# jthies/i-emic

Hardware: AMD Instinct MI355X
Metric: Newton-step wall time + SpMV achieved HBM GB/s, 2deg global ocean (lower is better)
Workload: dtype f64

## Files before the change

i-emic_amd/csrc/active_set.hip:

```cpp
#include <algorithm>
#include <vector>

#include "gs_internal.h"

namespace iemic {

namespace {

__global__ void k_cell_active(const uint8_t* __restrict__ known, Lay L, uint8_t* __restrict__ act)
{
    OWNED_CELL;
    bool a = false;
#pragma unroll
    for (int r = 0; r < NUN; r++) a |= !known[NUN * cell + r];
    act[lc] = a ? 1 : 0;
}

}

__global__ void k_dyn_pack(const double* __restrict__ val, const int* __restrict__ act, int64_t nact,
                           int64_t nloc, double* __restrict__ dvb, int64_t n)
{
    const int64_t t = (int64_t)blockIdx.x * blockDim.x + threadIdx.x;
    if (t >= n) return;
    const int64_t blk = t >> 12, s = (t >> 6) & 63, l = t & 63, h = blk * 64 + l;
    dvb[t] = h < nact ? val[s * nloc + act[h]] : 0.0;
}

__global__ void k_spmv_pack(const double* __restrict__ val, const int* __restrict__ act,
                                const int* __restrict__ apos, const int4* __restrict__ atl, int64_t nact,
                                int64_t nloc, double* __restrict__ spc)
{
    const int64_t t = (int64_t)blockIdx.x * blockDim.x + threadIdx.x;
    if (t >= (int64_t)NSLOT * nact) return;
    const int64_t s = t / nact, a = t - s * nact;
    const int4 td = atl[2 * apos[a]];
    spc[(int64_t)NSLOT * td.z + s * td.w + (a - td.z)] = val[s * nloc + act[a]];
}

__global__ void k_known_diff(const double* __restrict__ val, Lay L, int64_t rowintcon,
                             const uint8_t* __restrict__ known, double* __restrict__ nd)
{
    OWNED_CELL;
    int diff = 0;
    for (int r = 0; r < NUN; r++) {
        bool id = val[(int64_t)ROW_BEGIN[r] * ncell + lc] == 1.0;
        for (int s = ROW_BEGIN[r] + 1; id && s < ROW_BEGIN[r + 1]; s++)
            id = val[(int64_t)s * ncell + lc] == 0.0;
        const uint8_t k = (id && NUN * cell + r != rowintcon) ? 1 : 0;
        diff += k != known[NUN * cell + r];
    }
    if (diff) atomicAdd(nd, (double)diff);
}

static int act_tiles(iemic_ctx* c, const std::vector<uint8_t>& h, const std::vector<int>& cm)
{
    ActiveSet& as = c->gs.act;
    int rc;
    const int nx = c->sub.nx, tpr = (nx + 63) / 64;
    const int64_t nrow = c->sub.nloc / nx;
    std::vector<int> tl, ap((size_t)as.nact, 0);
    for (int64_t row = 0; row < nrow; row++)
        for (int ti = 0; ti < tpr; ti++) {
            const int i0 = ti * 64, nc = std::min(64, nx - i0);
            int lo = -1, hi = -1;
            uint64_t mask = 0;
            for (int cc = 0; cc < nc; cc++)
                if (h[row * nx + i0 + cc]) {
                    if (lo < 0) lo = cc;
                    hi = cc;
                    mask |= (uint64_t)1 << cc;
                }
            if (lo < 0) continue;
            const int a0 = cm[row * nx + i0 + lo], na = cm[row * nx + i0 + hi] - a0 + 1;
            for (int a = a0; a < a0 + na; a++) ap[a] = (int)(tl.size() / 8);
            tl.insert(tl.end(), {(int)(row * tpr + ti), lo | (hi << 8), a0, na, (int)(uint32_t)mask,
                                 (int)(uint32_t)(mask >> 32), 0, 0});
        }
    as.natile = (int)(tl.size() / 8);
    if (as.atl.reserve(tl.size() + 8)) return IEMIC_ENOMEM;
    if (!tl.empty() && (rc = h2d(c, as.atl.p, tl.data(), sizeof(int) * tl.size()))) return rc;
    if (as.apos.reserve(ap.size() + 1)) return IEMIC_ENOMEM;
    if (!ap.empty() && (rc = h2d(c, as.apos.p, ap.data(), sizeof(int) * ap.size()))) return rc;
    return 0;
}

int act_build(iemic_ctx* c, bool* changed)
{
    BlockGS& gs = c->gs;
    ActiveSet& as = gs.act;
    int rc;
    *changed = false;
    if (as.actf.reserve(c->sub.nloc)) return IEMIC_ENOMEM;
    hipLaunchKernelGGL(k_cell_active, dim3(blocks_for(c->sub.nloc)), dim3(256), 0, c->stream, gs.known.p,
                       lay_of(c->sub), as.actf.p);
    std::vector<uint8_t> h((size_t)c->sub.nloc);
    if ((rc = d2h(c, h.data(), as.actf.p, h.size()))) return rc;
    if (h == as.act_h) return 0;
    std::vector<int> list;
    list.reserve(h.size());
    for (int64_t q = 0; q < c->sub.nloc; q++)
        if (h[q]) list.push_back((int)q);
    as.nact = (int64_t)list.size();
    if (as.act.reserve(list.size() + 1)) return IEMIC_ENOMEM;
    if (!list.empty() && (rc = h2d(c, as.act.p, list.data(), sizeof(int) * list.size()))) return rc;
    std::vector<int> cm((size_t)c->sub.nloc, -1);
    for (size_t q = 0; q < list.size(); q++) cm[list[q]] = (int)q;
    if (as.cmap.reserve(cm.size())) return IEMIC_ENOMEM;
    if ((rc = h2d(c, as.cmap.p, cm.data(), sizeof(int) * cm.size()))) return rc;
    as.ric = -1;
    if (c->rowintcon >= 0) {
        const int64_t cell = c->rowintcon / NUN - c->sub.own0;
        if (cell >= 0 && cell < c->sub.nloc && cm[cell] >= 0) as.ric = (int64_t)NUN * cm[cell] + c->rowintcon % NUN;
    }
    if ((rc = act_tiles(c, h, cm))) return rc;
    as.act_h.swap(h);
    as.gen++;
    *changed = true;
    return 0;
}

static int dyn_halo_coefs(iemic_ctx* c)
{
    ActiveSet& as = c->gs.act;
    const int64_t row = (int64_t)c->l * c->sub.nx, nloc = c->sub.nloc;
    constexpr int NDS = 64;
    if (as.dvh.n < (size_t)(NDS * 2 * row)) {
        if (as.dvh.alloc((size_t)(NDS * 2 * row))) return IEMIC_ENOMEM;
        HIP_OK(hipMemsetAsync(as.dvh.p, 0, sizeof(double) * as.dvh.n, c->stream));
    }
    double* v = c->d_val.p;
    const int so = c->sub.nb[2], no = c->sub.nb[3];
    std::vector<Msg> y;
    push_pair(y, so, no, Seg{v, 0, NDS, row, nloc}, Seg{as.dvh.p, row, NDS, row, 2 * row},
              Seg{v, nloc - row, NDS, row, nloc}, Seg{as.dvh.p, 0, NDS, row, 2 * row});
    return run_msgs(c, y);
}

static int act_pack_dvb(iemic_ctx* c)
{
    ActiveSet& as = c->gs.act;
    if (as.nact <= 0 || !as.act.p) return 0;
    const int64_t nb = (as.nact + 63) / 64;
    if (as.dvb.reserve((size_t)(nb * 64 * 64))) return IEMIC_ENOMEM;
    hipLaunchKernelGGL(k_dyn_pack, dim3(blocks_for(nb * 64 * 64)), dim3(256), 0, c->stream, c->d_val.p,
                       (const int*)as.act.p, as.nact, c->sub.nloc, as.dvb.p, nb * 64 * 64);
    HIP_OK(hipGetLastError());
    return 0;
}

static int gs_pack_spc(iemic_ctx* c)
{
    ActiveSet& as = c->gs.act;
    if (as.nact <= 0 || !as.act.p) return 0;
    if (as.spc.reserve((size_t)(NSLOT * as.nact))) return IEMIC_ENOMEM;
    hipLaunchKernelGGL(k_spmv_pack, dim3(blocks_for(NSLOT * as.nact)), dim3(256), 0, c->stream, c->d_val.p,
                       (const int*)as.act.p, (const int*)as.apos.p, (const int4*)as.atl.p, as.nact, c->sub.nloc,
                       as.spc.p);
    HIP_OK(hipGetLastError());
    return 0;
}

int act_pack_streams(iemic_ctx* c)
{
    ActiveSet& as = c->gs.act;
    int rc;
    if (c->sub.nranks > 1 && c->sub.npx == 1 && (rc = dyn_halo_coefs(c))) return rc;
    if ((rc = act_pack_dvb(c))) return rc;
    if ((rc = gs_pack_spc(c))) return rc;
    as.vp = c->d_val.p;
    as.coef_stale = 0;
    as.cmp_ok = 1;
    return 0;
}

int gs_refresh(iemic_ctx* c)
{
    BlockGS& gs = c->gs;
    ActiveSet& as = gs.act;
    if (!as.coef_stale || !gs.ready || gs.kind != 2) return 0;
    as.coef_stale = 0;
    if (as.chk.reserve(1)) return IEMIC_ENOMEM;
    HIP_OK(hipMemsetAsync(as.chk.p, 0, sizeof(double), c->stream));
    hipLaunchKernelGGL(k_known_diff, dim3((unsigned)((c->sub.nloc + 255) / 256)), dim3(256), 0, c->stream,
                       c->d_val.p, lay_of(c->sub), (int64_t)c->rowintcon, gs.known.p, as.chk.p);
    int rc = allreduce_sum(c, as.chk.p, 1);
    if (rc) return rc;
    double nd = 0.0;
    if ((rc = d2h(c, &nd, as.chk.p, sizeof(double)))) return rc;
    if (nd != 0.0) as.cmp_ok = 0;
    return gs_pack_spc(c);
}

}
```

i-emic_amd/csrc/common.h:

```cpp
#ifndef IEMIC_COMMON_H
#define IEMIC_COMMON_H

#include <hip/hip_runtime.h>

#include <algorithm>
#include <cstdint>
#include <cstdio>
#include <string>
#include <vector>

#include "../../include/iemic.h"
#include "stencil.h"
#include "host_setup.h"
#include "decomp.h"

namespace iemic {

void set_error(const std::string& s);

#define HIP_OK(expr)                                                                   \
    do {                                                                               \
        hipError_t e_ = (expr);                                                        \
        if (e_ != hipSuccess) {                                                        \
            ::iemic::set_error(std::string(#expr) + ": " + hipGetErrorString(e_));     \
// ... 19 lines not shown
    }
    void free()
    {
        if (p) (void)hipFree(p);
        p = nullptr;
        n = 0;
    }
    DevBuf() = default;
    DevBuf(const DevBuf&) = delete;
    DevBuf& operator=(const DevBuf&) = delete;
    DevBuf(DevBuf&& o) noexcept : p(o.p), n(o.n) { o.p = nullptr; o.n = 0; }
    DevBuf& operator=(DevBuf&& o) noexcept
    {
        if (this != &o) {
            free();
            p = o.p; n = o.n;
            o.p = nullptr; o.n = 0;
        }
        return *this;
    }
    ~DevBuf() { free(); }
};

struct CrGemm {
    double* C;
    const double *C0, *C0b, *A1, *B1, *A2, *B2;
    double s1, s2;
};
constexpr int CR_MT = 8;
struct CrOut {
    int yb, nt;
    int64_t yo;
    double s[CR_MT];
    const double* A[CR_MT];
    int vb[CR_MT];
    int64_t vo[CR_MT];
};
struct CrComp {
    double* C;
    int nt;
    const double* A[4];
    const double* B[4];
    double s[4];
};
constexpr int CR_NCLS = 8;
struct CrCls {
    int ncls;
    int w0[CR_NCLS + 1];
    int nA[CR_NCLS];
    int64_t p0[CR_NCLS];
};
struct CrWg {
    int yref, r0;
    int nv, hasid;
    int vref[CR_MT];
};
struct CrPack {
    const double* A;
    double s;
    int64_t dst;
    int r0;
};
struct CrStep {
    int nwg = 0, rc = 16;
    int nl = 1;
    CrCls cls{};
    DevBuf<CrWg> wg;
    DevBuf<double> P;
    DevBuf<CrPack> jobs;
    int njobs = 0;
};
struct SchurCR {
    int n = 0, m = 0, periodic = 0, nlev = 0;
    std::vector<CrStep> down, up;
    DevBuf<double> cmat;
    DevBuf<CrComp> cdesc;
    int ncomp = 0;
    std::vector<int> N, per, merge;
    std::vector<size_t> dlr_off;
    std::vector<size_t> ap_off;
    std::vector<size_t> v_off;
    std::vector<int> g_off, g_cnt;
    int lt = 0, tM = 0;
    std::vector<size_t> tb_off;
    DevBuf<double> dlr, ap, bv, xv;
    DevBuf<double> tinv, tb, tx;
    DevBuf<CrGemm> gd;
    DevBuf<int> info;
};
int cr_init(iemic_ctx* c, SchurCR& cr, int n, int m, int periodic, int tail_max = 0);
int cr_factor(iemic_ctx* c, SchurCR& cr, const double* S9, const int* col_of_ij);
int cr_factor_blocks(iemic_ctx* c, SchurCR& cr);
int cr_check(iemic_ctx* c, SchurCR& cr);
int cr_solve(iemic_ctx* c, const SchurCR& cr, const double* b, double* x, hipStream_t s, double* xT = nullptr);
int cr_inverse_dev(hipStream_t s, int m, const double* src, double* dst, int* info);
int cr_inverse(hipStream_t s, int m, int count, const double* src, int s0, int sstep, double* dst, int* info);

struct TsMg {
    static constexpr int MAX = 12;
    int sweeps = 1, nlev = 0;
    int n[MAX] = {}, m[MAX] = {};
    int par[MAX] = {};
    DevBuf<double> off[MAX], diag[MAX], fac[MAX], b[MAX], z[MAX];
    DevBuf<double> zu[MAX];
    DevBuf<double> cinv;
    int glob = 0, gN = 0, gGX = 0, gI0 = 0, gJ0 = 0;
    DevBuf<double> gX, gband, gvec, gtmp, glpan;
    DevBuf<int> gpiv, ginfo, gcols;
    DevBuf<double> cdense;
    static constexpr int CR_CELLS = 1024;
    int crd = 0;
    int ckind = 0;
    bool nofuse = false;
    DevBuf<double> ep;
    DevBuf<uint64_t> etl;
    int64_t egen = -1, epn = 0;
    bool nopack = false;
    int hr = 0;
    SchurCR cr;
    DevBuf<int> cinfo;
};
int ts_mg_setup(iemic_ctx* c, int sweeps);
int ts_mg_solve(iemic_ctx* c, const double* zd, double* z, bool out, bool side);
int ts_mg_out(iemic_ctx* c, double* z);
int ts_mg_entry(iemic_ctx* c, const double* zd);
struct TsMgProbe {
    int nlev, lanes, sweeps, hr, ckind;
    int n, m, par, colours, fused, halo;
    const double *off, *diag, *b, *z, *cinv;
};
int ts_mg_probe(iemic_ctx* c, int q, TsMgProbe* o);

constexpr int BAND_NBP = 16;
int band_lu_inverse(iemic_ctx* c, double* ab, int N, int bl, int bu, int* piv, int* info_d, double* lpan,
                    const int* cols, double* X, int* info);

struct ActiveSet {
    DevBuf<int> act;
    DevBuf<int> cmap;
    int64_t ric = -1;
    DevBuf<uint8_t> actf;
    int64_t nact = 0;
    std::vector<uint8_t> act_h;
    int64_t gen = 0;
    DevBuf<double> spc;
    DevBuf<int> atl;
    DevBuf<int> apos;
    int natile = 0;
    DevBuf<double> dvh;
    DevBuf<double> dvb;
    const double* vp = nullptr;
    DevBuf<double> vold;
    int coef_stale = 0;
    int cmp_ok = 0;
    DevBuf<double> chk;
};
int act_build(iemic_ctx* c, bool* changed);
int act_pack_streams(iemic_ctx* c);
int gs_refresh(iemic_ctx* c);

struct TsSweeps {
    DevBuf<double> tsinv;
    DevBuf<double> tsoff;
    DevBuf<double> tsc, tic, bc;
    DevBuf<double> zt, zs;
    DevBuf<double> bts;
};

struct BlockGS {
    int ready = 0;
    int kind = 0;
    int ts_sweeps = 3;
    DevBuf<double> dinv;
    TsMg mg;
    ActiveSet act;
    TsSweeps sw;
    DevBuf<double> flags_d;
    std::vector<double> flags_h;
    DevBuf<int> own_pos;
    DevBuf<int> ocol;
    DevBuf<double> gslot;
    DevBuf<double> rcol;
    DevBuf<uint8_t> known;
    DevBuf<int> col_of_ij;
    DevBuf<int> ij_of_col;
    DevBuf<uint8_t> pinned;
    DevBuf<double> uvinv;
    DevBuf<double> tsdiag;
    DevBuf<double> pw;
    DevBuf<uint64_t> kmask;
    DevBuf<double> S9;
    SchurCR cr;
    int dyn_iters = 1;
    DevBuf<double> dres, zc;
    DevBuf<double> dq, dzero, dmr;
    int dyn_mr = 0;
    double dyn_omega = 1.0;
    int ts_at = 0;
    int schur_passes = 0;
    int ts_mg = 1;
    DevBuf<uint8_t> knP;
    DevBuf<double> zP, rrP;
    DevBuf<double> colvT;
    DevBuf<double> colvZ;
    DevBuf<double> rr, colv, colv2, colv_own;
};

struct Krylov {
    int m = 0;
    DevBuf<double> V, Z;
    DevBuf<double> w, r;
    int mc = 0;
    int64_t nc = 0;
    DevBuf<double> Vc, rf, t, bp;
    int zclean = 0;
};

struct Theta {
    double theta = 1.0, dt = 0.0;
    int init = 0;
    DevBuf<double> xold, Fold;
    DevBuf<double> Ft, b;
};

struct Eigs {
    int active = 0;
    int m = 0, j = 0;
    int broke = 0;
    double sigma = 0.0;
    DevBuf<double> V;
    DevBuf<double> t, w;
    DevBuf<double> lo;
};

constexpr int RED_BLOCKS = 1024;
__host__ __device__ inline double nanmax(double v, double a) { return (a > v || a != a) ? a : v; }
__device__ inline double block_nanmax(double v, double* sm)
{
    for (int o = 32; o > 0; o >>= 1) v = nanmax(v, __shfl_down(v, o, 64));
    if ((threadIdx.x & 63) == 0) sm[threadIdx.x >> 6] = v;
    __syncthreads();
    if (threadIdx.x == 0) {
        v = sm[0];
        for (int w = 1; w < 4; w++) v = nanmax(v, sm[w]);
    }
    return v;
}
constexpr int MAX_KRYLOV = 1000;
constexpr int RED_ROWS = 2 * MAX_KRYLOV + 8;
constexpr int DCGS_SCAL = 2 * MAX_KRYLOV + 2;

}

struct iemic_ctx {
    iemic_grid cfg;
    int device = 0;
    hipStream_t stream = nullptr;
    hipStream_t side = nullptr;
    hipEvent_t ev_fork = nullptr, ev_join = nullptr;
    int serial_setup = 0;
    int n = 0, m = 0, l = 0;
    int64_t ncell = 0, nrows = 0;
    int64_t rowintcon = -1;
    double int_correction = 0.0;
    void* comm = nullptr;
    void* group = nullptr;
    iemic_transport tp{};
    iemic::DevBuf<double> d_stage;
    std::vector<double> h_stage;
    int64_t stat[4] = {0, 0, 0, 0};
    double comm_timeout_s = 300.0;
    int comm_checked = 0;
    iemic::host::Setup su;
    const iemic::Sub& sub = su;
    iemic::DevBuf<int> d_landm;
    iemic::DevBuf<double> d_tab;
    iemic::DevBuf<double> d_ftab;
    iemic::DevBuf<double> d_frc;
    iemic::DevBuf<double> d_qcor;
    iemic::DevBuf<double> d_intc;
    iemic::DevBuf<double> d_atm;
    iemic::DevBuf<double> d_ins;
    int ins_on[4] = {0, 0, 0, 0};
    iemic::DevBuf<double> d_x, d_F, d_B, d_val;
    iemic::DevBuf<double> d_tmp1, d_tmp2, d_red;
    iemic::DevBuf<double> d_part, d_hbuf;
    double* h_red = nullptr;
    int jac_valid = 0;
    int refs = 1;
    iemic::BlockGS gs;
    iemic::Krylov kr;
    iemic::Theta th;
    iemic::Eigs eg;
    iemic::Geo geo() const;
    iemic_ctx() = default;
    iemic_ctx(const iemic_ctx&) = delete;
    iemic_ctx& operator=(const iemic_ctx&) = delete;
    ~iemic_ctx();
};

namespace iemic {
int dev_wait(iemic_ctx* c, hipEvent_t e, const char* what);
#define DEV_SYNC(c)                                                     \
    do {                                                                \
        const int rs_ = ::iemic::dev_wait((c), nullptr, __func__);      \
        if (rs_) return rs_;                                            \
    } while (0)
#define DEV_WAIT_EVENT(c, e)                                            \
    do {                                                                \
        const int rs_ = ::iemic::dev_wait((c), (e), __func__);          \
        if (rs_) return rs_;                                            \
    } while (0)
// ... 174 lines not shown
```

i-emic_amd/csrc/krylov.hip:

```cpp
#include <algorithm>
#include <cstdlib>
#include <chrono>
#include <cmath>

#include <hip/hip_ext.h>

#include "common.h"
#include "hessenberg.h"
#include "krylov_internal.h"
#include "vec_kernels.h"

namespace iemic {

__global__ void k_zero(double* __restrict__ p, int64_t n)
{
    for (int64_t q = (int64_t)blockIdx.x * blockDim.x + threadIdx.x; q < n; q += (int64_t)gridDim.x * blockDim.x)
        p[q] = 0.0;
}

__global__ void __launch_bounds__(256) k_mupdate_norm(const double* __restrict__ V, int64_t ldv,
                                                      int nvec, const double* __restrict__ h,
                                                      double* __restrict__ w, int64_t N,
                                                      double* __restrict__ partial)
{
// ... 337 lines not shown
        x[q] = acc;
    }
}

int mdot_host(iemic_ctx* c, const double* V, int64_t ldv, int nvec, const double* w,
              double* out, const double* ea, const double* eb)
{
    const int64_t N = c->sub.nlrows();
    const int nout = nvec + (ea ? 1 : 0);
    hipLaunchKernelGGL(k_mdot, dim3(RED_BLOCKS, nout), dim3(256), 0, c->stream, V, ldv, nvec, w, N,
                       c->d_part.p, ea, eb);
    hipLaunchKernelGGL(k_mdot_final, dim3(nout), dim3(256), 0, c->stream, c->d_part.p, RED_BLOCKS,
                       nout, c->d_hbuf.p);
    int rc = allreduce_sum(c, c->d_hbuf.p, nout);
    if (rc) return rc;
    HIP_OK(hipMemcpyAsync(c->h_red, c->d_hbuf.p, sizeof(double) * nout, hipMemcpyDeviceToHost,
                          c->stream));
    DEV_SYNC(c);
    for (int i = 0; i < nout; i++) out[i] = c->h_red[i];
    return 0;
}

int dot_owned(iemic_ctx* c, const double* a, const double* b, double* out)
{
    const int64_t o = owned(c).o;
    return mdot_host(c, a + o, 0, 1, b + o, out);
}

double dot(iemic_ctx* c, const double* a, const double* b, int64_t)
{
    const int64_t o = owned(c).o;
    double r = 0.0;
    if (mdot_host(c, a + o, 0, 1, b + o, &r)) return NAN;
    return r;
}

static int orth_pass(iemic_ctx* c, const double* V, int64_t ldv, int nvec, double* w, double* h,
                     double* ww0, double* ww1)
{
    const int64_t N = c->sub.nlrows();
    hipLaunchKernelGGL(k_mdot, dim3(RED_BLOCKS, nvec + 1), dim3(256), 0, c->stream, V, ldv, nvec,
                       w, N, c->d_part.p, (const double*)w);
    hipLaunchKernelGGL(k_mdot_final, dim3(nvec + 1), dim3(256), 0, c->stream, c->d_part.p,
                       RED_BLOCKS, nvec + 1, c->d_hbuf.p);
    int rc = allreduce_sum(c, c->d_hbuf.p, nvec + 1);
    if (rc) return rc;
    hipLaunchKernelGGL(k_mupdate_norm, dim3(RED_BLOCKS), dim3(256), 0, c->stream, V, ldv, nvec,
                       c->d_hbuf.p, w, N, c->d_part.p);
    hipLaunchKernelGGL(k_mdot_final, dim3(1), dim3(256), 0, c->stream, c->d_part.p, RED_BLOCKS, 1,
                       c->d_hbuf.p + nvec + 1);
    if ((rc = allreduce_sum(c, c->d_hbuf.p + nvec + 1, 1))) return rc;
    HIP_OK(hipMemcpyAsync(c->h_red, c->d_hbuf.p, sizeof(double) * (nvec + 2), hipMemcpyDeviceToHost,
                          c->stream));
    DEV_SYNC(c);
    for (int i = 0; i < nvec; i++) h[i] = c->h_red[i];
    *ww0 = c->h_red[nvec];
    *ww1 = c->h_red[nvec + 1];
    return 0;
}

int ensure_krylov(iemic_ctx* c, int m, int64_t nc)
{
    Krylov& k = c->kr;
    const int64_t N = c->sub.nerows();
    int rc = 0;
    if (k.m < m || !k.Z.p) {
        k.zclean = 0;
        k.V.free();
        rc |= k.Z.alloc((size_t)m * N);
        rc |= k.w.alloc(N);
        rc |= k.r.alloc(N);
        if (rc) {
            set_error("fgmres: out of device memory for the Krylov basis");
            return IEMIC_ENOMEM;
        }
        k.m = m;
    }
    if (!nc && !k.V.p) {
        if (k.V.alloc((size_t)(k.m + 1) * N)) {
            set_error("fgmres: out of device memory for the Krylov basis");
            return IEMIC_ENOMEM;
        }
    }
    if (nc && (k.mc < m || k.nc < nc || !k.Vc.p)) {
        rc |= k.Vc.alloc((size_t)(m + 1) * nc);
        if (!k.t.p) rc |= k.t.alloc(N) | k.bp.alloc(N);
        if (rc) {
            set_error("fgmres: out of device memory for the Krylov basis");
            return IEMIC_ENOMEM;
        }
        k.mc = m;
        k.nc = nc;
    }
    return 0;
}

__global__ void k_cgather(const double* __restrict__ full, const int* __restrict__ act, int64_t nc,
                          int64_t own0, double s, double* __restrict__ cmp)
{
    for (int64_t q = (int64_t)blockIdx.x * blockDim.x + threadIdx.x; q < nc;
         q += (int64_t)gridDim.x * blockDim.x) {
        const int64_t cl = q / NUN;
        cmp[q] = s * full[NUN * (own0 + act[cl]) + (q - NUN * cl)];
    }
}
__global__ void k_known_part(const double* __restrict__ v, const uint8_t* __restrict__ known, int64_t n0,
                             int64_t nl, double* __restrict__ t)
{
    for (int64_t q = (int64_t)blockIdx.x * blockDim.x + threadIdx.x; q < nl;
         q += (int64_t)gridDim.x * blockDim.x) {
        const int64_t r = n0 + q;
        t[r] = known[r] ? v[r] : 0.0;
    }
}

int upload_coeffs(iemic_ctx* c, const double* h, int n)
{
    if (n > RED_ROWS) {
        set_error("upload_coeffs: too many coefficients");
        return IEMIC_EINVAL;
    }
    double* st = c->h_red + RED_ROWS;
    for (int i = 0; i < n; i++) st[i] = h[i];
    HIP_OK(hipMemcpyAsync(c->d_hbuf.p + RED_ROWS, st, sizeof(double) * n,
                          hipMemcpyHostToDevice, c->stream));
    return 0;
}

int nonfinite()
{
    set_error("FGMRES: non-finite value in the Krylov basis (operator or preconditioner output)");
    return IEMIC_ERANGE;
}

double ms_since(std::chrono::steady_clock::time_point t0)
{
    return std::chrono::duration<double, std::milli>(std::chrono::steady_clock::now() - t0).count();
}

int prec_safeguard(iemic_ctx* c);

constexpr double STAG_RATIO = 0.25;
constexpr int STAG_MIN = 20;

int fgmres(iemic_ctx* c, const double* b, double* x, const iemic_krylov* opt, iemic_solve_info* info)
{
    const int m = std::max(1, std::min(opt->krylov_dim, MAX_KRYLOV));
    const Owned ow = owned(c);
    const int64_t NE = c->sub.nerows(), o = ow.o, NL = ow.n;
    const BlockGS& gs = c->gs;
    int rc = opt->prec > 0 ? gs_refresh(c) : 0;
    if (rc) return rc;
    const bool cmp = opt->orth == 0 && opt->prec == 2 && gs.ready && gs.kind == 2 && gs.act.nact > 0 && gs.act.cmap.p &&
                     gs.act.cmp_ok && gs.act.spc.p && gs.act.atl.p;
    const int64_t NC = cmp ? NUN * gs.act.nact : 0;
    rc = ensure_krylov(c, m, NC);
    if (rc) return rc;
    if (cmp && c->kr.zclean < m) {
        const int z0 = c->kr.zclean;
        if ((rc = dev_zero(c, c->kr.Z.p + (int64_t)z0 * NE, (int64_t)(m - z0) * NE))) return rc;
        c->kr.zclean = m;
    } else if (!cmp) {
        c->kr.zclean = 0;
    }
    iemic_solve_info inf{};
    auto T0 = std::chrono::steady_clock::now();
    double* V = cmp ? nullptr : c->kr.V.p;
    double* Vc = cmp ? c->kr.Vc.p : nullptr;
    double* Z = c->kr.Z.p;
    double* w = c->kr.w.p;
    double* r = c->kr.r.p;
    const unsigned G = ow.grid;
    const unsigned GC = grid_for(NC);
    Hessenberg hess(m);
    std::vector<double> h(m + 1), h2(m + 1), y(m);
    std::vector<double> zs(m + 1, 1.0);
    if (2 * m + 5 > RED_ROWS) {
        set_error("fgmres: Krylov dimension too large");
        return IEMIC_EINVAL;
    }
    int inf_reorth = 0;
    struct Events {
        hipEvent_t e[8] = {};
        ~Events() { for (auto& x : e) if (x) (void)hipEventDestroy(x); }
    } evs;
    hipEvent_t* ev = evs.e;
    hipEvent_t* evr = evs.e + 6;
    for (int q = 0; q < 6; q++) HIP_OK(hipEventCreate(&ev[q]));
    for (int q = 6; q < 8; q++) HIP_OK(hipEventCreateWithFlags(&evs.e[q], hipEventDisableTiming));

    if ((rc = dev_zero(c, x, NE))) return rc;
    double bnorm = sqrt0(dot(c, b, b, 0));
    if (!std::isfinite(bnorm)) return nonfinite();
    if (!(bnorm > 0)) {
        inf.converged = 1;
        if (info) *info = inf;
        return 0;
    }
    const double* b_orig = b;
    bool known_rhs = false;
    if (cmp) {
        double* t = c->kr.t.p;
        hipLaunchKernelGGL(k_known_part, dim3(G), dim3(256), 0, c->stream, b, gs.known.p, o, NL, t);
        if (dot(c, t, t, 0) > 0.0) {
            known_rhs = true;
            if ((rc = spmv(c, t, w, c->stream))) return rc;
            hipLaunchKernelGGL(k_axpby, dim3(G), dim3(256), 0, c->stream, 1.0, b + o, -1.0, w + o,
                               c->kr.bp.p + o, NL);
            b = c->kr.bp.p;
        }
    }
    HIP_OK(hipMemcpyAsync(r, b, sizeof(double) * NE, hipMemcpyDeviceToDevice, c->stream));
    double beta = known_rhs ? sqrt0(dot(c, b, b, 0)) : bnorm, res = beta / bnorm, res_c0 = res;
    int it = 0;
    struct Restore {
        iemic_ctx* c;
        int mr;
        ~Restore() { c->gs.dyn_mr = mr; }
    } restore{c, c->gs.dyn_mr};
    for (int cycle = 0; beta > 0.0 && cycle <= opt->max_restarts; cycle++) {
        const int it_c0 = it;
        if (cmp)
            hipLaunchKernelGGL(k_cgather, dim3(GC), dim3(256), 0, c->stream, r, gs.act.act.p, NC, c->sub.own0,
                               1.0 / beta, Vc);
        else
            hipLaunchKernelGGL(k_scale_copy, dim3(G), dim3(256), 0, c->stream, r + o, 1.0 / beta, V + o, NL);
        hess.reset(beta);
        int j = 0;
        if (opt->orth == 1) {
            for (; j < m; j++) {
                double* vj = V + (int64_t)j * NE;
                double* zj = Z + (int64_t)j * NE;
                double* vn = V + (int64_t)(j + 1) * NE;
                HIP_OK(hipEventRecord(ev[0], c->stream));
                if (opt->prec > 0) {
                    rc = prec_apply(c, vj, zj);
                    if (rc) return rc;
                } else {
                    HIP_OK(hipMemcpyAsync(zj, vj, sizeof(double) * NE, hipMemcpyDeviceToDevice, c->stream));
                }
                HIP_OK(hipEventRecord(ev[1], c->stream));
                rc = spmv(c, zj, vn, c->stream);
                if (rc) return rc;
                HIP_OK(hipEventRecord(ev[2], c->stream));

                double hn2 = 0.0;
                {
                    double ww0 = 0.0;
                    rc = orth_pass(c, V + o, NE, j + 1, vn + o, h.data(), &ww0, &hn2);
                    if (rc) return rc;
                    if (hn2 < 0.5 * ww0) {
                        double dummy = 0.0;
                        rc = orth_pass(c, V + o, NE, j + 1, vn + o, h2.data(), &dummy, &hn2);
                        if (rc) return rc;
                        for (int i = 0; i <= j; i++) h[i] += h2[i];
                        inf_reorth++;
                    }
                }
                if (!std::isfinite(hn2)) return nonfinite();
                double hn = sqrt0(hn2);
                if (hn > 0)
                    hipLaunchKernelGGL(k_scale_copy, dim3(G), dim3(256), 0, c->stream, vn + o, 1.0 / hn,
                                       vn + o, NL);
                {
                    float a1 = 0.f, a2 = 0.f;
                    (void)hipEventElapsedTime(&a1, ev[0], ev[1]);
                    (void)hipEventElapsedTime(&a2, ev[1], ev[2]);
                    inf.t_prec_ms += a1;
                    inf.t_spmv_ms += a2;
                    inf.n_spmv++;
                }
                res = hess.push_column(j, h.data(), hn) / bnorm;
                it++;
                if (res <= opt->tol || hn == 0.0) {
                    j++;
                    break;
                }
            }
        } else {
            std::vector<double> htent(m + 1), col(m + 1);
            int ncolf = 0;
            double* const Q = cmp ? Vc : V + o;
            const int64_t LQ = cmp ? NC : NE, NQ = cmp ? NC : NL;
            const int nbx1 = (int)std::min<int64_t>(RED_BLOCKS, (NQ / 2 + 256 * DOT1_E - 1) / (256 * DOT1_E));
            std::fill(zs.begin(), zs.end(), 1.0);
            auto enqueue = [&](int jj) -> int {
                double* u = Q + (int64_t)jj * LQ;
                double* wv = jj < m ? Q + (int64_t)(jj + 1) * LQ : nullptr;
                hipEvent_t* e = ev + 3 * (jj & 1);
                int rc2;
                if (jj < m) {
                    double* zj = Z + (int64_t)jj * NE;
                    HIP_OK(hipEventRecord(e[0], c->stream));
                    if (cmp) {
                        if ((rc2 = gs_apply_c(c, u, zj, jj > 0))) return rc2;
                    } else if (opt->prec > 0) {
                        if ((rc2 = prec_apply(c, u - o, zj))) return rc2;
                    } else {
                        HIP_OK(hipMemcpyAsync(zj, u - o, sizeof(double) * NE, hipMemcpyDeviceToDevice,
                                              c->stream));
                    }
                    if (cmp) {
                        if ((rc2 = halo_exchange(c, zj, 1))) return rc2;
                        if ((rc2 = spmv_kernel_c(c, zj, wv, e[1], e[2]))) return rc2;
                    } else {
                        HIP_OK(hipEventRecord(e[1], c->stream));
                        if ((rc2 = spmv(c, zj, wv - o, c->stream))) return rc2;
// ... 113 lines not shown
```

i-emic_amd/csrc/spmv.hip:

```cpp
#include <algorithm>
#include <cstdlib>

#include <hip/hip_ext.h>

#include "common.h"
#include "vec_kernels.h"

namespace iemic {

constexpr int SP7_T = 64;
__host__ __device__ constexpr int sp7_row(int s)
{
    return s < 24 ? 0 : s < 46 ? 1 : s < 53 ? 2 : s < 64 ? 3 : s < 84 ? 4 : 5;
}
__host__ __device__ constexpr int sp7_combo(int dj, int dk)
{
    return dk == 0 ? (dj + 1) : (dk == -1 ? (dj == 0 ? 3 : 5) : 4);
}
template <int S0, int S1>
__device__ __forceinline__ void sp7_load(const double* __restrict__ val, int64_t nloc, int64_t lc, bool act,
                                         double* v)
{
    if (act) {
#pragma unroll
        for (int s = S0; s < S1; s++) v[s - S0] = __builtin_nontemporal_load(val + (int64_t)s * nloc + lc);
    }
}
template <int S0, int S1>
__device__ __forceinline__ void sp7_compute(const double* v, const double* xs, int c, double* acc)
{
#pragma unroll
    for (int s = S0; s < S1; s++) {
        const Slot sl = SLOTS[s];
        const int q = sp7_combo(sl.dj, sl.dk);
        acc[sp7_row(s) - sp7_row(S0)] += v[s - S0] * xs[(q * (SP7_T + 2) + (c + 1 + sl.di)) * NUN + sl.var];
    }
}
__global__ void __launch_bounds__(256) k_spmv7(SubLay X, const double* __restrict__ val,
                                               const double* __restrict__ x,
                                               double* __restrict__ y, int nloc, int ntile, int tpr)
{
    __shared__ double xs[6 * (SP7_T + 2) * NUN];
    __shared__ double red[4][3][SP7_T];
    const int l = X.l, nx = X.nx;
    const int per = (ntile + 7) >> 3;
    const int tile = (int)(blockIdx.x & 7) * per + (int)(blockIdx.x >> 3);
    if (tile >= ntile) return;
    const int row = tile / tpr, i0 = (tile - row * tpr) * SP7_T;
    const int k = row % l, jl = row / l, j = X.jb0 + jl;
    const int nc = min(SP7_T, nx - i0);
    const int lc0 = row * nx + i0;
    const int t = threadIdx.x, c = t & 63;
    const int g = __builtin_amdgcn_readfirstlane(t >> 6);
    const bool act = c < nc;
    const int64_t lc = lc0 + c;
    double acc[3] = {0.0, 0.0, 0.0};
    double v[26];
    if (g == 0) sp7_load<0, 26>(val, nloc, lc, act, v);
    else if (g == 1) sp7_load<26, 52>(val, nloc, lc, act, v);
    else if (g == 2) sp7_load<52, 78>(val, nloc, lc, act, v);
    else sp7_load<78, 104>(val, nloc, lc, act, v);
    {
        const int jm = j > 0 ? j - 1 : j, jp = j < X.m - 1 ? j + 1 : j;
        const int km = k > 0 ? k - 1 : k, kp = k < l - 1 ? k + 1 : k;
        const int rj[6] = {jm, j, jp, j, j, jp}, rk[6] = {k, k, k, km, kp, km};
        constexpr int PR = (SP7_T + 2) * NUN;
        constexpr int SPT = (6 * PR + 255) / 256;
        const int lim = (nc + 2) * NUN;
        double xv[SPT];
        int xo[SPT];
#pragma unroll
        for (int u = 0; u < SPT; u++) {
            const int e = t + 256 * u;
            const int q = e / PR, w = e - q * PR;
            xo[u] = -1;
            if (e < 6 * PR && w < lim) {
                const int p = w / NUN, var = w - p * NUN;
                const int64_t r = (int64_t)(rj[q] - X.jb0 + HALO) * l + rk[q];
                const int64_t cell = (p == 0 || p == nc + 1)
                                         ? xnb_cell(r, i0 + p - 1, X.n, X.ib0, nx, X.hx, X.periodic, X.xb)
                                         : r * nx + i0 + p - 1;
                xo[u] = e;
                xv[u] = x[NUN * cell + var];
            }
        }
#pragma unroll
        for (int u = 0; u < SPT; u++)
            if (xo[u] >= 0) xs[xo[u]] = xv[u];
    }
    __syncthreads();
    if (g == 0) sp7_compute<0, 26>(v, xs, c, acc);
    else if (g == 1) sp7_compute<26, 52>(v, xs, c, acc);
    else if (g == 2) sp7_compute<52, 78>(v, xs, c, acc);
    else sp7_compute<78, 104>(v, xs, c, acc);
#pragma unroll
    for (int q = 0; q < 3; q++) red[g][q][c] = acc[q];
    __syncthreads();
    for (int o = t; o < nc * NUN; o += 256) {
        const int cc = o / NUN, R = o - cc * NUN;
        double v;
        switch (R) {
        case 0: v = red[0][0][cc]; break;
        case 1: v = red[0][1][cc] + red[1][0][cc]; break;
        case 2: v = red[1][1][cc] + red[2][0][cc]; break;
        case 3: v = red[2][1][cc]; break;
        case 4: v = red[2][2][cc] + red[3][0][cc]; break;
        default: v = red[3][1][cc]; break;
        }
        y[NUN * ((int64_t)HALO * l * nx + lc0) + o] = v;
    }
}

typedef __attribute__((address_space(3))) void lds_void;
typedef __attribute__((address_space(1))) void glb_void;
__global__ void __launch_bounds__(256) k_spmv7c(SubLay X, const double* __restrict__ spc,
                                                const double* __restrict__ x, double* __restrict__ y,
                                                const int4* __restrict__ atl, int natile, int tpr)
{
    __shared__ double xs[6 * (SP7_T + 2) * NUN];
    __shared__ double red[4][3][SP7_T];
    __shared__ int lof[SP7_T];
    const int l = X.l, nx = X.nx;
    const int per = (natile + 7) >> 3;
    const int pos = (int)(blockIdx.x & 7) * per + (int)(blockIdx.x >> 3);
    if (pos >= natile) return;
    const int4 td = atl[2 * pos], tm = atl[2 * pos + 1];
    const int tile = td.x, clo = td.y & 255, chi = td.y >> 8, a0 = td.z;
    const uint64_t amask = (uint64_t)(uint32_t)tm.x | ((uint64_t)(uint32_t)tm.y << 32);
    const int row = tile / tpr, i0 = (tile - row * tpr) * SP7_T;
    const int k = row % l, jl = row / l, j = X.jb0 + jl;
    const int nc = min(SP7_T, nx - i0);
    const int t = threadIdx.x, c = t & 63;
    const int g = __builtin_amdgcn_readfirstlane(t >> 6);
    const bool act = (amask >> c) & 1;
    const int cm = act ? a0 + __builtin_popcountll(amask & ((1ull << c) - 1)) : -1;
    if (g == 0 && act) lof[cm - a0] = c;
    double acc[3] = {0.0, 0.0, 0.0};
    double v[26];
    const double* vb = spc + (int64_t)NSLOT * a0;
    const int64_t vs = td.w, vo = cm - a0;
    if (g == 0) sp7_load<0, 26>(vb, vs, vo, act, v);
    else if (g == 1) sp7_load<26, 52>(vb, vs, vo, act, v);
    else if (g == 2) sp7_load<52, 78>(vb, vs, vo, act, v);
    else sp7_load<78, 104>(vb, vs, vo, act, v);
    {
        const int jm = j > 0 ? j - 1 : j, jp = j < X.m - 1 ? j + 1 : j;
        const int km = k > 0 ? k - 1 : k, kp = k < l - 1 ? k + 1 : k;
        const int rj[6] = {jm, j, jp, j, j, jp}, rk[6] = {k, k, k, km, kp, km};
        const int lane = t & 63, nb = nc * NUN * 8;
        const int blo = max(0, (clo - 1) * NUN * 8), bhi = min(nb, (chi + 2) * NUN * 8);
        for (int u = g; u < 18; u += 4) {
            const int q = u / 3, h = u - 3 * q;
            if (h * 1024 >= bhi || (h + 1) * 1024 <= blo) continue;
            const int byte = h * 1024 + lane * 16;
            const int64_t r = (int64_t)(rj[q] - X.jb0 + HALO) * l + rk[q];
            if (byte < nb)
                __builtin_amdgcn_global_load_lds((glb_void*)(x + NUN * (r * nx + i0) + byte / 8),
                                                 (lds_void*)(xs + (q * (SP7_T + 2) + 1) * NUN + h * 128), 16, 0, 0);
    }
        if (t < 72) {
            const int q = t / 12, side = (t / NUN) & 1, var = t - NUN * (t / NUN);
            const int p = side ? nc + 1 : 0;
            const int64_t r = (int64_t)(rj[q] - X.jb0 + HALO) * l + rk[q];
            const int64_t cell = xnb_cell(r, i0 + p - 1, X.n, X.ib0, nx, X.hx, X.periodic, X.xb);
            xs[(q * (SP7_T + 2) + p) * NUN + var] = x[NUN * cell + var];
    }
    }
    __syncthreads();
    if (act) {
        if (g == 0) sp7_compute<0, 26>(v, xs, c, acc);
        else if (g == 1) sp7_compute<26, 52>(v, xs, c, acc);
        else if (g == 2) sp7_compute<52, 78>(v, xs, c, acc);
        else sp7_compute<78, 104>(v, xs, c, acc);
    }
#pragma unroll
    for (int q = 0; q < 3; q++) red[g][q][c] = acc[q];
    __syncthreads();
    const int na = td.w;
    for (int o = t; o < na * NUN; o += 256) {
        const int ac = o / NUN, R = o - ac * NUN;
        const int cc = lof[ac];
        double vv;
        switch (R) {
        case 0: vv = red[0][0][cc]; break;
        case 1: vv = red[0][1][cc] + red[1][0][cc]; break;
        case 2: vv = red[1][1][cc] + red[2][0][cc]; break;
        case 3: vv = red[2][1][cc]; break;
        case 4: vv = red[2][2][cc] + red[3][0][cc]; break;
        default: vv = red[3][1][cc]; break;
        }
        y[(int64_t)NUN * a0 + o] = vv;
    }
}

template <int S0, int S1>
__device__ __forceinline__ void dyn_partial(const double* __restrict__ val, const double* __restrict__ z,
                                            int64_t vs, const int (*nc)[9], const bool* on,
                                            int64_t ps, double* acc)
{
    constexpr int NS = S1 - S0;
    double v[NS], zz[NS];
#pragma unroll
    for (int s = 0; s < NS; s++) v[s] = zz[s] = 0.0;
#pragma unroll
    for (int q = 0; q < 2; q++) {
        if (!on[q]) continue;
#pragma unroll
        for (int s = S0; s < S1; s++) {
            const Slot sl = SLOTS[s];
            if (sp7_row(s) - sp7_row(S0) != q) continue;
            const int cidx = nc[sl.di + 1][(sl.dk + 1) * 3 + (sl.dj + 1)];
            v[s - S0] = val[(int64_t)s * vs];
            zz[s - S0] = z[(int64_t)cidx + ps * sl.var];
        }
    }
#pragma unroll
    for (int s = S0; s < S1; s++) {
        const int q = sp7_row(s) - sp7_row(S0);
        if (on[q]) acc[q] += v[s - S0] * zz[s - S0];
    }
}
__global__ void __launch_bounds__(256) __attribute__((amdgpu_waves_per_eu(5, 8))) k_spmv_dyn(SubLay X, const double* __restrict__ val,
                                                  const double* __restrict__ z,
                                                  const double* __restrict__ r,
                                                  const uint8_t* __restrict__ knP,
                                                  double* __restrict__ d, int64_t nloc, int nblk, int64_t ps,
                                                  const double* __restrict__ hv, int nhb, int hs, int hn,
                                                  const int* __restrict__ alist, int64_t nown,
                                                  const double* __restrict__ vb)
{
    __shared__ double red[4][2][64];
    __shared__ int64_t us[64];
    __shared__ int oks[64];
    const int ntot = nblk + nhb;
    const int per = (ntot + 7) >> 3;
    const int tile = (int)(blockIdx.x & 7) * per + (int)(blockIdx.x >> 3);
    if (tile >= ntot) return;
    const int c = threadIdx.x & 63, g = threadIdx.x >> 6;
    const int64_t row = (int64_t)X.l * X.nx;
    const int64_t e0 = (int64_t)HALO * row;
    const bool halo = tile >= nblk;
    int64_t h, u;
    bool act;
    if (!halo) {
        h = (int64_t)tile * 64 + c;
        act = h < nown;
        u = !act ? 0 : (alist ? (int64_t)alist[h] : h);
    } else {
        h = (int64_t)(tile - nblk) * 64 + c;
        const bool south = h < row;
        act = h < 2 * row && (south ? hs : hn);
        u = south ? h - row : nloc + h - row;
    }
    if (g == 0) {
        us[c] = u;
        oks[c] = act ? 1 : 0;
    }
    double acc[2] = {0.0, 0.0};
    if (act) {
        const int64_t q = u + row;
        const int il = (int)(q % X.nx), k = (int)((q / X.nx) % X.l);
        const int j = X.jb0 - 1 + (int)(q / row);
        int nc[3][9];
        nb_cells(X, il, j, k, nc);
        const int64_t cell = e0 + u;
        const int v0 = g == 0 ? 0 : g - 1;
        const bool on[2] = {!knP[cell + ps * v0], g > 0 && !knP[cell + ps * (v0 + 1)]};
        const double* vp = halo ? hv + h : (vb ? vb + (int64_t)tile * 4096 + c : val + u);
        const int64_t vs = halo ? 2 * row : (vb ? 64 : nloc);
        if (g == 0) dyn_partial<0, 16>(vp, z, vs, nc, on, ps, acc);
        else if (g == 1) dyn_partial<16, 32>(vp, z, vs, nc, on, ps, acc);
        else if (g == 2) dyn_partial<32, 48>(vp, z, vs, nc, on, ps, acc);
        else dyn_partial<48, 64>(vp, z, vs, nc, on, ps, acc);
    }
    red[g][0][c] = acc[0];
    red[g][1][c] = acc[1];
    __syncthreads();
    const int R = threadIdx.x >> 6, cc = threadIdx.x & 63;
    if (!oks[cc]) return;
    const double sum = R == 0 ? red[0][0][cc] + red[1][0][cc]
                     : R == 1 ? red[1][1][cc] + red[2][0][cc]
                     : R == 2 ? red[2][1][cc] + red[3][0][cc]
                              : red[3][1][cc];
    const int64_t cell = e0 + us[cc], e = cell + ps * R;
    d[e] = knP[e] ? 0.0 : r[e] - sum;
}

int spmv_dyn_defect(iemic_ctx* c, const double* z, const double* r, const uint8_t* knP, double* d, bool halo)
{
    const BlockGS& gs = c->gs;
    const bool al = gs.act.act.p && gs.act.nact > 0;
    const int64_t nown = al ? gs.act.nact : c->sub.nloc;
    const int nblk = (int)((nown + 63) / 64);
    const int64_t row = (int64_t)c->l * c->sub.nx;
    const bool hv = halo && gs.act.dvh.p;
    const int nhb = hv ? (int)((2 * row + 63) / 64) : 0;
    const unsigned grid = 8u * (unsigned)((nblk + nhb + 7) / 8);
    hipLaunchKernelGGL(k_spmv_dyn, dim3(grid), dim3(256), 0, c->stream, sub_lay(c->sub), gs.act.vp, z, r, knP, d,
                       c->sub.nloc, nblk, (int64_t)c->sub.next, hv ? gs.act.dvh.p : nullptr, nhb,
                       hv && c->sub.nb[2] >= 0 ? 1 : 0, hv && c->sub.nb[3] >= 0 ? 1 : 0,
                       al ? gs.act.act.p : nullptr, nown, al && gs.act.dvb.p ? gs.act.dvb.p : nullptr);
    return 0;
}

static int spmv_intcond(iemic_ctx* c, const double* x, double* yr);
int spmv_kernel(iemic_ctx* c, const double* x, double* y)
{
    if (!c->jac_valid) {
        set_error("spmv: no Jacobian assembled");
        return IEMIC_ESTATE;
    }
    hipStream_t s = c->stream;
    if (c->sub.nloc >= INT32_MAX) {
        set_error("spmv: more than 2^31 cells per rank");
        return IEMIC_EINVAL;
    }
    const int tpr = (c->sub.nx + SP7_T - 1) / SP7_T;
    const int ntile = (int)(c->sub.nloc / c->sub.nx) * tpr;
    const unsigned grid = 8u * (unsigned)((ntile + 7) / 8);
    hipLaunchKernelGGL(k_spmv7, dim3(grid), dim3(256), 0, s, sub_lay(c->sub), c->d_val.p, x, y, (int)c->sub.nloc, ntile,
                       tpr);
    return spmv_intcond(c, x, c->rowintcon >= 0 ? y + c->rowintcon : nullptr);
}

static int spmv_intcond(iemic_ctx* c, const double* x, double* yr)
{
    hipStream_t s = c->stream;
    if (c->su.rowintcon_ref >= 0) {
        const Owned w = owned(c);
        hipLaunchKernelGGL(k_mdot, dim3(RED_BLOCKS, 1), dim3(256), 0, s, c->d_intc.p + w.o, (int64_t)0, 1,
                           x + w.o, w.n, c->d_red.p);
        hipLaunchKernelGGL(k_mdot_final, dim3(1), dim3(256), 0, s, c->d_red.p, RED_BLOCKS, 1,
                           c->d_red.p + RED_BLOCKS);
        int rc = allreduce_sum(c, c->d_red.p + RED_BLOCKS, 1);
        if (rc) return rc;
        if (c->rowintcon >= 0)
            hipLaunchKernelGGL(k_scale_copy, dim3(1), dim3(1), 0, s, c->d_red.p + RED_BLOCKS,
                               (double)c->cfg.int_sign, yr, (int64_t)1);
    }
    HIP_OK(hipGetLastError());
    return 0;
}

int spmv_kernel_c(iemic_ctx* c, const double* x, double* yc, hipEvent_t ev0, hipEvent_t ev1)
{
    const BlockGS& gs = c->gs;
    if (!c->jac_valid || !gs.act.cmap.p || !gs.act.spc.p || !gs.act.atl.p || gs.act.coef_stale) {
        set_error("spmv: no Jacobian, no active-cell map or stale packed coefficients");
        return IEMIC_ESTATE;
    }
    hipStream_t s = c->stream;
    const int tpr = (c->sub.nx + SP7_T - 1) / SP7_T;
    const unsigned grid = 8u * (unsigned)((gs.act.natile + 7) / 8);
    if (gs.act.natile > 0)
        hipExtLaunchKernelGGL(k_spmv7c, dim3(grid), dim3(256), 0, s, ev0, ev1, 0, sub_lay(c->sub),
                              (const double*)gs.act.spc.p, x, yc, (const int4*)gs.act.atl.p, gs.act.natile, tpr);
    double* yr = nullptr;
    if (c->rowintcon >= 0) {
        if (c->gs.act.ric < 0) {
            set_error("spmv: the integral-condition row lies in an inactive cell");
            return IEMIC_EINVAL;
        }
        yr = yc + c->gs.act.ric;
    }
    return spmv_intcond(c, x, yr);
}

int spmv(iemic_ctx* c, double* x, double* y, hipStream_t)
{
    int rc = halo_exchange(c, x, 1);
    if (rc) return rc;
    return spmv_kernel(c, x, y);
}

}
```

Measured before the change: 99.34.

## Share dynamics coefficient block between GS dvb buffer and compact SpMV stream

During Jacobian setup the compact SpMV coefficient buffer now stores only slots 64..NSLOT-1. The first 64 dynamics slots are read from the already-packed dvb buffer used by the Gauss-Seidel preconditioner. This shrinks the spc footprint and the pack kernel's traffic, and may let the two streams share cache residency. The cost is a second, differently laid out read stream in k_spmv7c with strided dvb accesses. It also adds state (spc_shared/spc_own) that must stay consistent across refreshes.

```diff
diff --git a/i-emic_amd/csrc/active_set.hip b/i-emic_amd/csrc/active_set.hip
--- a/i-emic_amd/csrc/active_set.hip
+++ b/i-emic_amd/csrc/active_set.hip
@@ -29,13 +29,13 @@
 
 __global__ void k_spmv_pack(const double* __restrict__ val, const int* __restrict__ act,
                                 const int* __restrict__ apos, const int4* __restrict__ atl, int64_t nact,
-                                int64_t nloc, double* __restrict__ spc)
+                                int64_t nloc, double* __restrict__ spc, int s0, int ns)
 {
     const int64_t t = (int64_t)blockIdx.x * blockDim.x + threadIdx.x;
-    if (t >= (int64_t)NSLOT * nact) return;
+    if (t >= (int64_t)ns * nact) return;
     const int64_t s = t / nact, a = t - s * nact;
     const int4 td = atl[2 * apos[a]];
-    spc[(int64_t)NSLOT * td.z + s * td.w + (a - td.z)] = val[s * nloc + act[a]];
+    spc[(int64_t)ns * td.z + s * td.w + (a - td.z)] = val[(s0 + s) * nloc + act[a]];
 }
 
 __global__ void k_known_diff(const double* __restrict__ val, Lay L, int64_t rowintcon,
@@ -149,15 +149,21 @@
     return 0;
 }
 
-static int gs_pack_spc(iemic_ctx* c)
-{
-    ActiveSet& as = c->gs.act;
+static int gs_pack_spc(iemic_ctx* c, bool setup_jac)
+{
+    ActiveSet& as = c->gs.act;
+    as.spc_shared = 0;
     if (as.nact <= 0 || !as.act.p) return 0;
-    if (as.spc.reserve((size_t)(NSLOT * as.nact))) return IEMIC_ENOMEM;
-    hipLaunchKernelGGL(k_spmv_pack, dim3(blocks_for(NSLOT * as.nact)), dim3(256), 0, c->stream, c->d_val.p,
+    const bool sh = setup_jac && !as.spc_own && as.dvb.p;
+    constexpr int NDYN = ROW_BEGIN[TT];
+    static_assert(NDYN == 64, "dvb holds slots 0..63, 64 per block row");
+    const int s0 = sh ? NDYN : 0, ns = NSLOT - s0;
+    if (as.spc.reserve((size_t)ns * (size_t)as.nact)) return IEMIC_ENOMEM;
+    hipLaunchKernelGGL(k_spmv_pack, dim3(blocks_for((int64_t)ns * as.nact)), dim3(256), 0, c->stream, c->d_val.p,
                        (const int*)as.act.p, (const int*)as.apos.p, (const int4*)as.atl.p, as.nact, c->sub.nloc,
-                       as.spc.p);
+                       as.spc.p, s0, ns);
     HIP_OK(hipGetLastError());
+    as.spc_shared = sh ? 1 : 0;
     return 0;
 }
 
@@ -167,7 +173,7 @@
     int rc;
     if (c->sub.nranks > 1 && c->sub.npx == 1 && (rc = dyn_halo_coefs(c))) return rc;
     if ((rc = act_pack_dvb(c))) return rc;
-    if ((rc = gs_pack_spc(c))) return rc;
+    if ((rc = gs_pack_spc(c, true))) return rc;
     as.vp = c->d_val.p;
     as.coef_stale = 0;
     as.cmp_ok = 1;
@@ -189,7 +195,16 @@
     double nd = 0.0;
     if ((rc = d2h(c, &nd, as.chk.p, sizeof(double)))) return rc;
     if (nd != 0.0) as.cmp_ok = 0;
-    return gs_pack_spc(c);
-}
-
-}
+    return gs_pack_spc(c, false);
+}
+
+int act_force_own(iemic_ctx* c, int own)
+{
+    BlockGS& gs = c->gs;
+    ActiveSet& as = gs.act;
+    as.spc_own = own ? 1 : 0;
+    if (!gs.ready || gs.kind != 2 || as.coef_stale) return 0;
+    return gs_pack_spc(c, as.vp == c->d_val.p);
+}
+
+}
diff --git a/i-emic_amd/csrc/common.h b/i-emic_amd/csrc/common.h
--- a/i-emic_amd/csrc/common.h
+++ b/i-emic_amd/csrc/common.h
@@ -195,12 +195,19 @@
     const double* vp = nullptr;
     DevBuf<double> vold;
     int coef_stale = 0;
+    int spc_shared = 0;
+    int spc_own = 0;
     int cmp_ok = 0;
     DevBuf<double> chk;
 };
+inline bool act_spmv_streams(const ActiveSet& as)
+{
+    return as.spc.p && as.atl.p && (!as.spc_shared || as.dvb.p);
+}
 int act_build(iemic_ctx* c, bool* changed);
 int act_pack_streams(iemic_ctx* c);
 int gs_refresh(iemic_ctx* c);
+int act_force_own(iemic_ctx* c, int own);
 
 struct TsSweeps {
     DevBuf<double> tsinv;
diff --git a/i-emic_amd/csrc/krylov.hip b/i-emic_amd/csrc/krylov.hip
--- a/i-emic_amd/csrc/krylov.hip
+++ b/i-emic_amd/csrc/krylov.hip
@@ -513,7 +513,7 @@
     int rc = opt->prec > 0 ? gs_refresh(c) : 0;
     if (rc) return rc;
     const bool cmp = opt->orth == 0 && opt->prec == 2 && gs.ready && gs.kind == 2 && gs.act.nact > 0 && gs.act.cmap.p &&
-                     gs.act.cmp_ok && gs.act.spc.p && gs.act.atl.p;
+                     gs.act.cmp_ok && act_spmv_streams(gs.act);
     const int64_t NC = cmp ? NUN * gs.act.nact : 0;
     rc = ensure_krylov(c, m, NC);
     if (rc) return rc;
diff --git a/i-emic_amd/csrc/spmv.hip b/i-emic_amd/csrc/spmv.hip
--- a/i-emic_amd/csrc/spmv.hip
+++ b/i-emic_amd/csrc/spmv.hip
@@ -34,6 +34,22 @@
         const Slot sl = SLOTS[s];
         const int q = sp7_combo(sl.dj, sl.dk);
         acc[sp7_row(s) - sp7_row(S0)] += v[s - S0] * xs[(q * (SP7_T + 2) + (c + 1 + sl.di)) * NUN + sl.var];
+    }
+}
+constexpr bool SP7C_DVB_NT = false;
+constexpr int SP7C_NDYN = 64;
+template <int S0, int S1, bool SH>
+__device__ __forceinline__ void sp7c_load(const double* __restrict__ run, int64_t na, int64_t vo,
+                                          const double* __restrict__ dv, bool act, double* v)
+{
+    if (act) {
+#pragma unroll
+        for (int s = S0; s < S1; s++) {
+            if (SH && s < SP7C_NDYN)
+                v[s - S0] = SP7C_DVB_NT ? __builtin_nontemporal_load(dv + s * 64) : dv[s * 64];
+            else
+                v[s - S0] = __builtin_nontemporal_load(run + (int64_t)(SH ? s - SP7C_NDYN : s) * na + vo);
+        }
     }
 }
 __global__ void __launch_bounds__(256) k_spmv7(SubLay X, const double* __restrict__ val,
@@ -113,7 +129,9 @@
 
 typedef __attribute__((address_space(3))) void lds_void;
 typedef __attribute__((address_space(1))) void glb_void;
+template <bool SH>
 __global__ void __launch_bounds__(256) k_spmv7c(SubLay X, const double* __restrict__ spc,
+                                                const double* __restrict__ dvb,
                                                 const double* __restrict__ x, double* __restrict__ y,
                                                 const int4* __restrict__ atl, int natile, int tpr)
 {
@@ -137,12 +155,13 @@
     if (g == 0 && act) lof[cm - a0] = c;
     double acc[3] = {0.0, 0.0, 0.0};
     double v[26];
-    const double* vb = spc + (int64_t)NSLOT * a0;
+    const double* vb = spc + (int64_t)(SH ? NSLOT - SP7C_NDYN : NSLOT) * a0;
     const int64_t vs = td.w, vo = cm - a0;
-    if (g == 0) sp7_load<0, 26>(vb, vs, vo, act, v);
-    else if (g == 1) sp7_load<26, 52>(vb, vs, vo, act, v);
-    else if (g == 2) sp7_load<52, 78>(vb, vs, vo, act, v);
-    else sp7_load<78, 104>(vb, vs, vo, act, v);
+    const double* dv = SH && act ? dvb + ((int64_t)(cm >> 6) * 4096 + (cm & 63)) : nullptr;
+    if (g == 0) sp7c_load<0, 26, SH>(vb, vs, vo, dv, act, v);
+    else if (g == 1) sp7c_load<26, 52, SH>(vb, vs, vo, dv, act, v);
+    else if (g == 2) sp7c_load<52, 78, SH>(vb, vs, vo, dv, act, v);
+    else sp7c_load<78, 104, SH>(vb, vs, vo, dv, act, v);
     {
         const int jm = j > 0 ? j - 1 : j, jp = j < X.m - 1 ? j + 1 : j;
         const int km = k > 0 ? k - 1 : k, kp = k < l - 1 ? k + 1 : k;
@@ -345,16 +364,23 @@
 int spmv_kernel_c(iemic_ctx* c, const double* x, double* yc, hipEvent_t ev0, hipEvent_t ev1)
 {
     const BlockGS& gs = c->gs;
-    if (!c->jac_valid || !gs.act.cmap.p || !gs.act.spc.p || !gs.act.atl.p || gs.act.coef_stale) {
+    if (!c->jac_valid || !gs.act.cmap.p || !act_spmv_streams(gs.act) || gs.act.coef_stale) {
         set_error("spmv: no Jacobian, no active-cell map or stale packed coefficients");
         return IEMIC_ESTATE;
     }
     hipStream_t s = c->stream;
     const int tpr = (c->sub.nx + SP7_T - 1) / SP7_T;
     const unsigned grid = 8u * (unsigned)((gs.act.natile + 7) / 8);
-    if (gs.act.natile > 0)
-        hipExtLaunchKernelGGL(k_spmv7c, dim3(grid), dim3(256), 0, s, ev0, ev1, 0, sub_lay(c->sub),
-                              (const double*)gs.act.spc.p, x, yc, (const int4*)gs.act.atl.p, gs.act.natile, tpr);
+    if (gs.act.natile > 0) {
+        if (gs.act.spc_shared)
+            hipExtLaunchKernelGGL(k_spmv7c<true>, dim3(grid), dim3(256), 0, s, ev0, ev1, 0, sub_lay(c->sub),
+                                  (const double*)gs.act.spc.p, (const double*)gs.act.dvb.p, x, yc,
+                                  (const int4*)gs.act.atl.p, gs.act.natile, tpr);
+        else
+            hipExtLaunchKernelGGL(k_spmv7c<false>, dim3(grid), dim3(256), 0, s, ev0, ev1, 0, sub_lay(c->sub),
+                                  (const double*)gs.act.spc.p, (const double*)nullptr, x, yc,
+                                  (const int4*)gs.act.atl.p, gs.act.natile, tpr);
+    }
     double* yr = nullptr;
     if (c->rowintcon >= 0) {
         if (c->gs.act.ric < 0) {
```

Result: no change. 98.61 (median of 3 runs) (-0.7%).
